# maryambabaei/hybrid-FEM-LSSVR

Measured on AMD Instinct MI355X. Metric: LSSVR-enhanced elements/sec, 1D Poisson deg-8/16-pt, higher is better.
Workload: dtype f64

## Files before the change

### __graft_entry__.py

```python
from __future__ import annotations

import os
import subprocess
import sys

ROOT = os.path.dirname(os.path.abspath(__file__))
if ROOT not in sys.path:
    sys.path.insert(0, ROOT)

CSRC = os.path.join(ROOT, "hybrid_fem_lssvr_amd", "csrc")


def build() -> None:
    if os.environ.get("LSSVR_HIP_LIB"):
        raise RuntimeError("LSSVR_HIP_LIB is set: build(), the tests and the benchmark use the one "
                           "in-tree library only (the override is for scripts/ A/B experiments)")
    env = dict(os.environ)
    env.setdefault("HIPCC", "/opt/rocm/bin/hipcc")
    subprocess.run(["make", "-C", CSRC, "-j", str(min(8, os.cpu_count() or 1))], check=True, env=env)
    subprocess.run(["make", "-C", CSRC, "demo"], check=True, env=env)
    subprocess.run(["make", "-C", CSRC, "check-dpp"], check=True, env=env)
    import hybrid_fem_lssvr_amd as pkg
    lib = pkg._capi.load()
    assert pkg._capi.LIB_PATH == pkg._capi.IN_TREE_LIB
    assert lib.lssvr_version() == pkg._capi.ABI_VERSION
    import oracle.lssvr_oracle


def smoke() -> None:
    import numpy as np
    import torch
    import hybrid_fem_lssvr_amd as pkg
    from oracle import lssvr_oracle as orc

    if not torch.cuda.is_available():
        raise RuntimeError("smoke() needs cuda:0 (MI355X); there is no CPU fallback")
    solver = pkg.FEMLSSVRPrimalSolver(25, lssvr_M=9, lssvr_gamma=1e4, global_domain=(-1, 1),
                                      n_colloc=16)
    solver.solve()
    nodes = np.linspace(-1, 1, 25)
    u_ref = orc.fem_p1_solve(nodes)
    assert np.max(np.abs(solver.fem_values - u_ref)) < 1e-13, "P1 solve mismatch"
    W = np.array([f.coef for f in solver.lssvr_functions])
    W_ref = orc.enhance_all_vec(nodes, solver.fem_values, 9, 1e4, 16)
    err = orc.rel_l2_coef(W, W_ref).max()
    assert err < 1e-12, f"enhance mismatch {err}"
    xq = np.linspace(-1, 1, 201)
    uq = solver.evaluate_solution(xq)
    uo, eo = orc.evaluate_solution(nodes, W, xq)
    assert np.max(np.abs(uq - uo)) < 1e-14, "evaluate mismatch"
    assert np.array_equal(solver.element_indices(xq), eo), "element index mismatch"
    l2 = np.linalg.norm(uq - orc.true_solution(xq)) / np.linalg.norm(orc.true_solution(xq))
    big = pkg.enhance_elements(nodes, solver.fem_values, 33, 1e4, n_colloc=64)
    Wb = big.W.cpu().numpy()
    Wb_ref = orc.enhance_all_vec(nodes, solver.fem_values, 33, 1e4, 64)
    errb = orc.rel_l2_coef(Wb, Wb_ref).max()
    assert errb < 1e-11, f"degree-32 mismatch {errb}"
    print(f"smoke ok: deg8 rel-L2 vs oracle {err:.2e}, deg32 {errb:.2e}, "
          f"hybrid rel-L2 error vs sin(pi x) {l2:.3e}")


if __name__ == "__main__":
    build()
    if len(sys.argv) > 1 and sys.argv[1] == "smoke":
        smoke()
```

### hybrid_fem_lssvr_amd/csrc/capi.hip

```cpp
#include <cstdarg>
#include <vector>
#include <cstdio>
#include <cstring>

#include <new>
#include "lssvr_kernels.hpp"

namespace {

thread_local char g_err[256] = {0};

int fail(int code, const char* fmt, ...) {
  va_list ap;
  va_start(ap, fmt);
  vsnprintf(g_err, sizeof(g_err), fmt, ap);
  va_end(ap);
  return code;
}

int check_launch(hipError_t e, const char* what) {
  if (e == hipSuccess) return LSSVR_OK;
  return fail(LSSVR_ERR_LAUNCH, "%s: %s", what, hipGetErrorString(e));
}

int check_ne(int64_t ne, int ne_min = 1, const char* why = "") {
  if (ne < ne_min) return fail(LSSVR_ERR_SIZE, "ne = %lld < %d%s", (long long)ne, ne_min, why);
  if (ne > (int64_t)1 << 40) return fail(LSSVR_ERR_SIZE, "ne = %lld too large", (long long)ne);
  return LSSVR_OK;
}

bool is_finite(double v) { return v > -INFINITY && v < INFINITY; }

int check_layout(int table_layout) {
  if (table_layout != LSSVR_TABLE_ELEMENT_MAJOR && table_layout != LSSVR_TABLE_POINT_MAJOR)
    return fail(LSSVR_ERR_SIZE, "unknown table_layout %d", table_layout);
  return LSSVR_OK;
}

int check_kinds(int kind_left, int kind_right) {
  if ((kind_left != LSSVR_END_DIRICHLET && kind_left != LSSVR_END_ROBIN) ||
      (kind_right != LSSVR_END_DIRICHLET && kind_right != LSSVR_END_ROBIN))
    return fail(LSSVR_ERR_SIZE, "end kinds (%d, %d) must be LSSVR_END_DIRICHLET or LSSVR_END_ROBIN", kind_left,
                kind_right);
  return LSSVR_OK;
}

int check_nl_kind(int kind, int nterm) {
  if (kind != LSSVR_NL_POLY && kind != LSSVR_NL_EXP)
    return fail(LSSVR_ERR_RHS, "unknown kind %d (LSSVR_NL_POLY or LSSVR_NL_EXP)", kind);
  if (kind == LSSVR_NL_POLY && (nterm < 1 || nterm > 6))
    return fail(LSSVR_ERR_SIZE, "nterm = %d outside [1, 6]", nterm);
  if (kind == LSSVR_NL_EXP && nterm != 2) return fail(LSSVR_ERR_SIZE, "nterm = %d: LSSVR_NL_EXP has q_0 and q_1", nterm);
  return LSSVR_OK;
}

int bind_enhance(lssvr::EnhanceArgs& a, const double* x, const double* u, int64_t ne, int64_t elem_offset,
                 int64_t ne_global, double gxmin, double gxmax, double bc_left, double bc_right, int M,
                 int n_colloc, double gamma, double* W, int32_t* status, int32_t* fail_count) {
  if (ne < 0) return fail(LSSVR_ERR_SIZE, "ne = %lld < 0", (long long)ne);
  if (ne > 0 && (!x || !u || !W)) return fail(LSSVR_ERR_NULL, "x, u and W must be non-NULL");
  if (elem_offset < 0 || ne_global < elem_offset + ne)
    return fail(LSSVR_ERR_SIZE, "shard [%lld, %lld) does not fit ne_global = %lld",
                (long long)elem_offset, (long long)(elem_offset + ne), (long long)ne_global);
  if (M < 2 || M > lssvr::kLargeMaxM)
    return fail(LSSVR_ERR_DEGREE, "M = %d outside [2, %d]", M, lssvr::kLargeMaxM);
  if (n_colloc < 2 || n_colloc > 4096)
    return fail(LSSVR_ERR_SIZE, "n_colloc = %d outside [2, 4096]", n_colloc);
  if (!(gamma > 0.0)) return fail(LSSVR_ERR_SIZE, "gamma must be > 0");
  if (ne * (int64_t)M / M != ne) return fail(LSSVR_ERR_SIZE, "ne*M overflows");
  a = lssvr::EnhanceArgs{};
  a.x = x;
  a.u = u;
  a.ne = ne;
  a.ne_mesh = ne;
  a.elem_offset = elem_offset;
  a.ne_global = ne_global;
  a.gxmin = gxmin;
  a.gxmax = gxmax;
  a.bc_left = bc_left;
  a.bc_right = bc_right;
  a.gamma = gamma;
  a.inv_gamma = 1.0 / gamma;
// ... 260 lines not shown

int colloc_points_entry(const double* x, int64_t ne, int n_colloc, double* xc, void* stream, bool point_major) {
  if (ne < 0) return fail(LSSVR_ERR_SIZE, "ne < 0");
  if (n_colloc < 2) return fail(LSSVR_ERR_SIZE, "n_colloc < 2");
  if (ne > 0 && (!x || !xc)) return fail(LSSVR_ERR_NULL, "x and xc must be non-NULL");
  return check_launch(lssvr::colloc_points(x, ne, n_colloc, xc, reinterpret_cast<hipStream_t>(stream), point_major),
                      point_major ? "colloc_points(point-major)" : "colloc_points");
}

}

extern "C" {

int lssvr_version(void) { return LSSVR_ABI_VERSION; }

const char* lssvr_last_error(void) { return g_err; }

int lssvr_enhance(const double* x, const double* u, int64_t ne, int64_t elem_offset,
                  int64_t ne_global, double gxmin, double gxmax, double bc_left, double bc_right,
                  int M, int n_colloc, double gamma, int rhs_id, const double* rhs_params_host,
                  const double* rhs_values, int solver_id, double* W, int32_t* status,
                  int32_t* fail_count, void* stream) {
  return lssvr_enhance_ws(x, u, ne, elem_offset, ne_global, gxmin, gxmax, bc_left, bc_right, M, n_colloc, gamma,
                          rhs_id, rhs_params_host, rhs_values, solver_id, W, status, fail_count, nullptr, 0, stream,
                          nullptr);
}

int64_t lssvr_enhance_work_bytes(int64_t ne, int M, int n_colloc, int solver_id) {
  if (ne <= 0) return 0;
  if (solver_id == LSSVR_SOLVER_PRIMAL_MOMENT) return lssvr::enhance_moment_ws_bytes(ne, M, n_colloc);
  if (solver_id != LSSVR_SOLVER_PRIMAL || M <= lssvr::kSmallMaxM) return 0;
  return lssvr::enhance_moment_ws_bytes(ne, M, n_colloc);
}

int lssvr_enhance_ws(const double* x, const double* u, int64_t ne, int64_t elem_offset,
                     int64_t ne_global, double gxmin, double gxmax, double bc_left, double bc_right,
                     int M, int n_colloc, double gamma, int rhs_id, const double* rhs_params_host,
                     const double* rhs_values, int solver_id, double* W, int32_t* status,
                     int32_t* fail_count, void* work, int64_t work_bytes, void* stream,
                     float* kernel_ms_host) {
  lssvr::EnhanceArgs a;
  const int rc = bind_enhance_ws(a, x, u, ne, elem_offset, ne_global, gxmin, gxmax, bc_left, bc_right, M, n_colloc,
                                 gamma, rhs_id, rhs_params_host, rhs_values, solver_id, W, status, fail_count, work,
                                 work_bytes);
  if (rc != LSSVR_OK || ne == 0) return rc;
  hipStream_t s = reinterpret_cast<hipStream_t>(stream);
  return timed_launch([&](const lssvr::LaunchOpts* o) { return enhance_dispatch(a, solver_id, s, o, work, work_bytes); },
                      kernel_ms_host);
}

int lssvr_enhance_ws_sequence(const double* x, const double* u, int64_t ne, int64_t elem_offset,
                              int64_t ne_global, double gxmin, double gxmax, double bc_left, double bc_right,
                              int M, int n_colloc, double gamma, int rhs_id, const double* rhs_params_host,
                              const double* rhs_values, int solver_id, double* W, int32_t* status,
                              int32_t* fail_count, void* work, int64_t work_bytes, void* stream,
                              int repeats, float* kernel_ms_host) {
  lssvr::EnhanceArgs a;
  int rc = check_sequence(ne, repeats, kernel_ms_host);
  if (rc == LSSVR_OK)
    rc = bind_enhance_ws(a, x, u, ne, elem_offset, ne_global, gxmin, gxmax, bc_left, bc_right, M, n_colloc, gamma,
                         rhs_id, rhs_params_host, rhs_values, solver_id, W, status, fail_count, work, work_bytes);
  if (rc != LSSVR_OK) return rc;
  hipStream_t s = reinterpret_cast<hipStream_t>(stream);
  return timed_sequence([&](const lssvr::LaunchOpts* o) { return enhance_dispatch(a, solver_id, s, o, work, work_bytes); },
                        s, repeats, kernel_ms_host);
}

int lssvr_enhance_profiled(const double* x, const double* u, int64_t ne, int64_t elem_offset,
                           int64_t ne_global, double gxmin, double gxmax, double bc_left,
                           double bc_right, int M, int n_colloc, double gamma, int rhs_id,
                           const double* rhs_params_host, const double* rhs_values, int solver_id,
                           double* W, int32_t* status, void* stream, float* kernel_ms_host) {
  if (!kernel_ms_host) return fail(LSSVR_ERR_NULL, "kernel_ms_host must be non-NULL");
  if (ne < 1) return fail(LSSVR_ERR_SIZE, "nothing to profile: ne = %lld", (long long)ne);
  return lssvr_enhance_ws(x, u, ne, elem_offset, ne_global, gxmin, gxmax, bc_left, bc_right, M, n_colloc, gamma,
                          rhs_id, rhs_params_host, rhs_values, solver_id, W, status, nullptr, nullptr, 0, stream,
                          kernel_ms_host);
}

struct lssvr_step_plan {
  lssvr::EnhanceArgs a;
  lssvr::P1Args p;
  const double* memo = nullptr;
};

static int64_t step_memo_bytes(const lssvr_step_plan& b) {
  const lssvr::EnhanceArgs& a = b.a;
  if (a.M > lssvr::kSmallMaxM || a.refine > 0 || a.gamma_values || a.rhs_id != LSSVR_RHS_SIN || a.ne < 1) return 0;
  return 8 * lssvr::step_memo_doubles(a.M, a.ne);
}

static int bind_step(lssvr_step_plan& b, const double* x, const double* u, int64_t ne, int64_t elem_offset,
                     int64_t ne_global, double gxmin, double gxmax, double bc_left, double bc_right,
                     int M, int n_colloc, double gamma, const double* rhs_params_host, int nquad,
                     double* diag, double* off, double* load, double* W, int32_t* status,
                     int32_t* fail_count) {
  lssvr::EnhanceArgs& a = b.a;
  int rc = bind_enhance(a, x, u, ne, elem_offset, ne_global, gxmin, gxmax, bc_left, bc_right, M, n_colloc, gamma,
                        W, status, fail_count);
  if (rc != LSSVR_OK) return rc;
  if (ne < 1) return fail(LSSVR_ERR_SIZE, "ne = %lld < 1", (long long)ne);
  rc = bind_p1(b.p, x, ne, nquad, diag, off, load);
  if (rc == LSSVR_OK) rc = bind_rhs(a, LSSVR_RHS_SIN, rhs_params_host, nullptr, false, "ne");
  if (rc != LSSVR_OK) return rc;
  if (n_colloc < M - 2)
    return fail(LSSVR_ERR_SOLVER, "lssvr_step: n_colloc = %d < M-2 = %d: the primal normal equations are "
                                  "rank deficient; use lssvr_p1_assemble + lssvr_enhance (dual solver)",
                n_colloc, M - 2);
  return bind_p1_rhs(b.p, LSSVR_RHS_SIN, rhs_params_host, nullptr);
}

static int run_step(const lssvr_step_plan& b, hipStream_t s) {
  const lssvr::EnhanceArgs& a = b.a;
  const lssvr::P1Args& p = b.p;
  if (a.M <= lssvr::kSmallMaxM && a.refine == 0)
    return check_launch(lssvr::step_small(a, p, s, nullptr, b.memo), "step_small");
  int rc = check_launch(lssvr::p1_assemble(p, s), "p1_assemble");
  if (rc != LSSVR_OK) return rc;
  if (a.M <= lssvr::kSmallMaxM) return check_launch(lssvr::enhance_small(a, s), "enhance_small(refine)");
  return check_launch(lssvr::enhance_large(a, s), "enhance_large");
}

int lssvr_step(const double* x, const double* u, int64_t ne, int64_t elem_offset,
               int64_t ne_global, double gxmin, double gxmax, double bc_left, double bc_right,
               int M, int n_colloc, double gamma, const double* rhs_params_host, int nquad,
               double* diag, double* off, double* load, double* W, int32_t* status,
               int32_t* fail_count, void* stream) {
  lssvr_step_plan b;
  const int rc = bind_step(b, x, u, ne, elem_offset, ne_global, gxmin, gxmax, bc_left, bc_right, M, n_colloc,
                           gamma, rhs_params_host, nquad, diag, off, load, W, status, fail_count);
  if (rc != LSSVR_OK) return rc;
  return run_step(b, reinterpret_cast<hipStream_t>(stream));
}

int lssvr_step_plan_create(lssvr_step_plan** plan, const double* x, const double* u, int64_t ne,
                           int64_t elem_offset, int64_t ne_global, double gxmin, double gxmax,
                           double bc_left, double bc_right, int M, int n_colloc, double gamma,
                           const double* rhs_params_host, int nquad, double* diag, double* off,
                           double* load, double* W, int32_t* status, int32_t* fail_count) {
  if (!plan) return fail(LSSVR_ERR_NULL, "plan must be non-NULL");
  *plan = nullptr;
  lssvr_step_plan* b = new (std::nothrow) lssvr_step_plan;
  if (!b) return fail(LSSVR_ERR_LAUNCH, "out of host memory");
  const int rc = bind_step(*b, x, u, ne, elem_offset, ne_global, gxmin, gxmax, bc_left, bc_right, M, n_colloc,
                           gamma, rhs_params_host, nquad, diag, off, load, W, status, fail_count);
  if (rc != LSSVR_OK) {
    delete b;
    return rc;
  }
  *plan = b;
  return LSSVR_OK;
}

int lssvr_step_plan_launch(const lssvr_step_plan* plan, void* stream) {
  if (!plan) return fail(LSSVR_ERR_NULL, "plan must be non-NULL");
  return run_step(*plan, reinterpret_cast<hipStream_t>(stream));
}

int64_t lssvr_step_plan_memo_bytes(const lssvr_step_plan* plan) { return plan ? step_memo_bytes(*plan) : 0; }

int lssvr_step_plan_memo_bind(lssvr_step_plan* plan, void* memo, int64_t memo_bytes, void* stream) {
  if (!plan) return fail(LSSVR_ERR_NULL, "plan must be non-NULL");
  if (!memo) {
    plan->memo = nullptr;
    return LSSVR_OK;
  }
  const int64_t need = step_memo_bytes(*plan);
  if (need == 0)
    return fail(LSSVR_ERR_SOLVER, "this plan cannot use a memo (lssvr_step_plan_memo_bytes is 0: M = %d, n_colloc = %d)",
                plan->a.M, plan->a.n);
  if (memo_bytes < need)
    return fail(LSSVR_ERR_SIZE, "memo_bytes = %lld < lssvr_step_plan_memo_bytes = %lld", (long long)memo_bytes,
                (long long)need);
  if (reinterpret_cast<uintptr_t>(memo) % 8 != 0) return fail(LSSVR_ERR_SIZE, "memo must be 8-byte aligned");
  plan->memo = nullptr;
  const int rc = check_launch(lssvr::step_small_memo_fill(plan->a, static_cast<double*>(memo),
                                                          reinterpret_cast<hipStream_t>(stream)),
                              "step_memo_fill");
  if (rc == LSSVR_OK) plan->memo = static_cast<const double*>(memo);
  return rc;
}

int lssvr_step_plan_destroy(lssvr_step_plan* plan) {
  delete plan;
  return LSSVR_OK;
}

int lssvr_enhance_varcoef(const double* x, const double* u, int64_t ne, int64_t elem_offset,
                          int64_t ne_global, double gxmin, double gxmax, double bc_left,
                          double bc_right, int M, int n_colloc, double gamma,
                          const double* a_values, const double* da_values,
                          const double* rhs_values, double* W, int32_t* status,
                          int32_t* fail_count, void* stream) {
  return lssvr_enhance_varcoef_ws(x, u, ne, elem_offset, ne_global, gxmin, gxmax, bc_left, bc_right, M,
                                  n_colloc, gamma, a_values, da_values, rhs_values, LSSVR_TABLE_ELEMENT_MAJOR,
                                  W, status, fail_count, nullptr, 0, stream, nullptr);
}

int lssvr_step_varcoef(const double* x, const double* u, int64_t ne, int64_t elem_offset,
                       int64_t ne_global, double gxmin, double gxmax, double bc_left, double bc_right,
                       int M, int n_colloc, double gamma, const double* a_values,
                       const double* da_values, const double* rhs_values, int table_layout, int nquad,
                       const double* rhs_quad, const double* a_quad, double* diag, double* off,
                       double* load, double* W, int32_t* status, int32_t* fail_count, void* stream) {
  lssvr::EnhanceArgs a;
  int rc = bind_enhance(a, x, u, ne, elem_offset, ne_global, gxmin, gxmax, bc_left, bc_right, M, n_colloc, gamma,
                        W, status, fail_count);
  if (rc != LSSVR_OK) return rc;
  if (ne < 1) return fail(LSSVR_ERR_SIZE, "ne = %lld < 1", (long long)ne);
  rc = bind_varcoef(a, a_values, da_values, rhs_values, table_layout, true);
  if (rc != LSSVR_OK) return rc;
  if (!rhs_quad || !a_quad) return fail(LSSVR_ERR_NULL, "rhs_quad and a_quad must be non-NULL");
  lssvr::P1Args p;
  rc = bind_p1(p, x, ne, nquad, diag, off, load);
  if (rc != LSSVR_OK) return rc;
  if (n_colloc < M - 2)
    return fail(LSSVR_ERR_SOLVER, "lssvr_step_varcoef: n_colloc = %d < M-2 = %d: use lssvr_p1_assemble + "
                                  "lssvr_enhance_varcoef (dual solver)", n_colloc, M - 2);
  p.rhs_id = LSSVR_RHS_ARRAY;
  p.rhs_quad = rhs_quad;
  p.a_quad = a_quad;
  hipStream_t s = reinterpret_cast<hipStream_t>(stream);
  if (M <= lssvr::kStepVarcoefFusedMaxM) return check_launch(lssvr::step_small_vc(a, p, s), "step_small_vc");
  rc = check_launch(lssvr::p1_assemble(p, s), "p1_assemble");
  if (rc != LSSVR_OK) return rc;
  return enhance_dispatch(a, LSSVR_SOLVER_PRIMAL, s, nullptr);
}

int lssvr_enhance_react(const double* x, const double* u, int64_t ne, int64_t elem_offset,
                        int64_t ne_global, double gxmin, double gxmax, double bc_left,
                        double bc_right, int M, int n_colloc, double gamma,
                        const double* a_values, const double* da_values, const double* c_values,
                        const double* rhs_values, double* W, int32_t* status,
                        int32_t* fail_count, void* stream) {
  return lssvr_enhance_react_ws(x, u, ne, elem_offset, ne_global, gxmin, gxmax, bc_left, bc_right, M,
                                n_colloc, gamma, a_values, da_values, c_values, rhs_values,
                                LSSVR_TABLE_ELEMENT_MAJOR, W, status, fail_count, nullptr, 0, stream, nullptr);
}

int lssvr_enhance_react_ws(const double* x, const double* u, int64_t ne, int64_t elem_offset,
                           int64_t ne_global, double gxmin, double gxmax, double bc_left,
                           double bc_right, int M, int n_colloc, double gamma,
                           const double* a_values, const double* da_values, const double* c_values,
                           const double* rhs_values, int table_layout, double* W, int32_t* status,
                           int32_t* fail_count, void* work, int64_t work_bytes, void* stream,
                           float* kernel_ms_host) {
  lssvr::EnhanceReactArgs a;
  const int rc = bind_react_ws(a, x, u, ne, elem_offset, ne_global, gxmin, gxmax, bc_left, bc_right, M, n_colloc,
                               gamma, a_values, da_values, c_values, rhs_values, table_layout, W, status,
                               fail_count, work, work_bytes);
  if (rc != LSSVR_OK || ne == 0) return rc;
  hipStream_t s = reinterpret_cast<hipStream_t>(stream);
  return timed_launch([&](const lssvr::LaunchOpts* o) { return react_dispatch(a, s, o); }, kernel_ms_host);
}

int lssvr_enhance_multi(const double* x, const double* u, int64_t ne, int64_t elem_offset,
                        int64_t ne_global, double gxmin, double gxmax, const double* bc_values, int ncases,
                        int M, int n_colloc, double gamma, const double* a_values, const double* da_values,
                        const double* c_values, const double* rhs_values, int table_layout, double* W,
                        int32_t* status, int32_t* fail_count, void* stream, float* kernel_ms_host) {
  lssvr::EnhanceMultiArgs a{};
  int rc = bind_varcoef_ws(a, x, u, ne, elem_offset, ne_global, gxmin, gxmax, 0.0, 0.0, M, n_colloc, gamma,
// ... 1332 lines not shown
```

### hybrid_fem_lssvr_amd/csrc/enhance_small.hip

```cpp
#include "lssvr_kernels.hpp"
#include "lssvr_p1.hpp"

namespace lssvr {

#define LSSVR_DECLARE_SMALL_RANGE(NAME)                                                          \
  hipError_t enhance_small_##NAME(const EnhanceArgs& a, hipStream_t s, const LaunchOpts* o);     \
  hipError_t step_small_##NAME(const EnhanceArgs& e, const P1Args& a, const QuadRule& q,         \
                               hipStream_t s, const LaunchOpts* o, const double* memo);          \
  hipError_t step_memo_fill_##NAME(const EnhanceArgs& e, double* memo, hipStream_t s);           \
  hipError_t step_small_vc_##NAME(const EnhanceArgs& e, const P1Args& a, const QuadRule& q,      \
                                  hipStream_t s, const LaunchOpts* o);
LSSVR_DECLARE_SMALL_RANGE(a)
LSSVR_DECLARE_SMALL_RANGE(b)
LSSVR_DECLARE_SMALL_RANGE(c)
LSSVR_DECLARE_SMALL_RANGE(d)

hipError_t enhance_small(const EnhanceArgs& a, hipStream_t s, const LaunchOpts* o) {
  if (a.M <= 10) return enhance_small_a(a, s, o);
  if (a.M <= 15) return enhance_small_b(a, s, o);
  if (a.M <= 19) return enhance_small_c(a, s, o);
  return enhance_small_d(a, s, o);
}

hipError_t step_small(const EnhanceArgs& e, const P1Args& a, hipStream_t s, const LaunchOpts* o,
                      const double* memo) {
  QuadRule q;
  if (!quad_rule(a.nquad, q)) return hipErrorInvalidValue;
  if (e.M <= 10) return step_small_a(e, a, q, s, o, memo);
  if (e.M <= 15) return step_small_b(e, a, q, s, o, memo);
  if (e.M <= 19) return step_small_c(e, a, q, s, o, memo);
  return step_small_d(e, a, q, s, o, memo);
}

hipError_t step_small_memo_fill(const EnhanceArgs& e, double* memo, hipStream_t s) {
  if (e.M <= 10) return step_memo_fill_a(e, memo, s);
  if (e.M <= 15) return step_memo_fill_b(e, memo, s);
  if (e.M <= 19) return step_memo_fill_c(e, memo, s);
  return step_memo_fill_d(e, memo, s);
}

hipError_t step_small_vc(const EnhanceArgs& e, const P1Args& a, hipStream_t s, const LaunchOpts* o) {
  QuadRule q;
  if (!quad_rule(a.nquad, q)) return hipErrorInvalidValue;
  if (e.M <= 10) return step_small_vc_a(e, a, q, s, o);
  if (e.M <= 15) return step_small_vc_b(e, a, q, s, o);
  return hipErrorInvalidValue;
}

}
```

### hybrid_fem_lssvr_amd/csrc/enhance_small_impl.hpp

```cpp
#pragma once
#include "enhance_small_cheb.hpp"
#include "lssvr_device.hpp"
#include "lssvr_kernels.hpp"
#include "lssvr_p1.hpp"

namespace lssvr {

constexpr int kStageK = 8;
constexpr int kStageArr = 64 * (kStageK + 1);
template <int M, int RHS, bool VC, bool RX = false>
constexpr int kSmallTilePerWave =
    (RHS == LSSVR_RHS_ARRAY && (VC ? (RX ? 4 : 3) : 1) * kStageArr > 64 * M) ? (VC ? (RX ? 4 : 3) : 1) * kStageArr
                                                                             : 64 * M;
constexpr int kPrefetch = 4;
constexpr int kPrefetchReact = 2;

template <int M, int RHS, bool VC, bool RX = false, typename Args = EnhanceArgs>
__device__ __forceinline__ void enhance_small_body(const Args& p, const unsigned block,
                                                   double* __restrict__ tile) {
  static_assert(!RX || VC, "reaction rows extend the variable-coefficient rows");
  constexpr int MR = M - 2;
  constexpr int NT = MR * (MR + 1) / 2;

  const int tid = threadIdx.x;
// ... 331 lines not shown
    if (i <= a.ne) p1_node<true>(a, q, i);
  }
}

template <int M>
__global__ __launch_bounds__(kBlock) void step_memo_fill_kernel(EnhanceArgs p, double* memo) {
  if constexpr (M == 2) {
    const int64_t e = (int64_t)blockIdx.x * kBlock + threadIdx.x;
    if (e < p.ne) {
      memo[e] = p.x[e];
      if (e == p.ne - 1) memo[e + 1] = p.x[e + 1];
    }
  } else {
    enhance_small_body_cheb<M, LSSVR_RHS_SIN, false, NoProbe, MemoFill>(p, blockIdx.x, nullptr, NoProbe{}, MemoFill{memo});
  }
}

constexpr int kStepVcMaxM = 12;
template <int M, int RHS>
__global__ __launch_bounds__(kBlock) void step_small_vc_kernel(EnhanceArgs p, P1Args a, QuadRule q,
                                                                unsigned eblocks) {
  __shared__ double tile[(kBlock / 64) * kSmallTilePerWave<M, RHS, true>];
  if (blockIdx.x < eblocks) {
    enhance_small_body<M, RHS, true>(p, blockIdx.x, tile);
  } else {
    const int64_t i = (int64_t)(blockIdx.x - eblocks) * kBlock + threadIdx.x;
    if (i <= a.ne) p1_node<false>(a, q, i);
  }
}

template <int M, int RHS, bool VC>
static hipError_t launch_small(const EnhanceArgs& a, hipStream_t s, const LaunchOpts* o) {
  const unsigned blocks = (unsigned)((a.ne + kBlock - 1) / kBlock);
  if constexpr (!VC && M >= kRefineMinM) {
    if (a.refine > 0) return launch(enhance_small_refine_kernel<M, RHS>, dim3(blocks), dim3(kBlock), s, o, a);
  }
  return launch(enhance_small_kernel<M, RHS, VC, 1>, dim3(blocks), dim3(kBlock), s, o, a);
}

template <int M>
static hipError_t launch_step(const EnhanceArgs& e, const P1Args& a, const QuadRule& q,
                              hipStream_t s, const LaunchOpts* o, const double* memo) {
  const unsigned eb = (unsigned)((e.ne + kBlock - 1) / kBlock);
  const unsigned ab = (unsigned)((a.ne + 1 + kBlock - 1) / kBlock);
  return launch(step_small_kernel<M>, dim3(eb + ab), dim3(kBlock), s, o, e, a, q, eb, memo);
}

template <int M>
static hipError_t launch_memo_fill(const EnhanceArgs& e, double* memo, hipStream_t s) {
  const unsigned eb = (unsigned)((e.ne + kBlock - 1) / kBlock);
  return launch(step_memo_fill_kernel<M>, dim3(eb), dim3(kBlock), s, nullptr, e, memo);
}

template <int M>
static hipError_t launch_step_vc(const EnhanceArgs& e, const P1Args& a, const QuadRule& q,
                                 hipStream_t s, const LaunchOpts* o) {
  if constexpr (M <= kStepVcMaxM) {
    const unsigned eb = (unsigned)((e.ne + kBlock - 1) / kBlock);
    const unsigned ab = (unsigned)((a.ne + 1 + kBlock - 1) / kBlock);
    if (e.tab_ps != 1)
      return launch(step_small_vc_kernel<M, LSSVR_RHS_ARRAY_PM>, dim3(eb + ab), dim3(kBlock), s, o, e, a, q, eb);
    return launch(step_small_vc_kernel<M, LSSVR_RHS_ARRAY>, dim3(eb + ab), dim3(kBlock), s, o, e, a, q, eb);
  } else {
    return hipErrorInvalidValue;
  }
}

#define LSSVR_DEFINE_SMALL_RANGE(NAME, FOR_EACH_M)                                              \
  hipError_t enhance_small_##NAME(const EnhanceArgs& a, hipStream_t s, const LaunchOpts* o) {    \
    switch (a.M) {                                                                               \
      FOR_EACH_M(LSSVR_SMALL_CASE_ENH)                                                           \
      default:                                                                                   \
        return hipErrorInvalidValue;                                                             \
    }                                                                                            \
  }                                                                                              \
  hipError_t step_small_##NAME(const EnhanceArgs& e, const P1Args& a, const QuadRule& q,         \
                               hipStream_t s, const LaunchOpts* o, const double* memo) {         \
    switch (e.M) {                                                                               \
      FOR_EACH_M(LSSVR_SMALL_CASE_STEP)                                                          \
      default:                                                                                   \
        return hipErrorInvalidValue;                                                             \
    }                                                                                            \
  }                                                                                              \
  hipError_t step_memo_fill_##NAME(const EnhanceArgs& e, double* memo, hipStream_t s) {          \
    switch (e.M) {                                                                               \
      FOR_EACH_M(LSSVR_SMALL_CASE_MEMO_FILL)                                                     \
      default:                                                                                   \
        return hipErrorInvalidValue;                                                             \
    }                                                                                            \
  }                                                                                              \
  hipError_t step_small_vc_##NAME(const EnhanceArgs& e, const P1Args& a, const QuadRule& q,      \
                                  hipStream_t s, const LaunchOpts* o) {                          \
    switch (e.M) {                                                                               \
      FOR_EACH_M(LSSVR_SMALL_CASE_STEP_VC)                                                       \
      default:                                                                                   \
        return hipErrorInvalidValue;                                                             \
    }                                                                                            \
  }

#define LSSVR_SMALL_CASE_ENH(MM)                                                     \
  case MM:                                                                           \
    if (a.a_values && a.tab_ps != 1) return launch_small<MM, LSSVR_RHS_ARRAY_PM, true>(a, s, o); \
    if (a.a_values) return launch_small<MM, LSSVR_RHS_ARRAY, true>(a, s, o);         \
    if (a.rhs_id == LSSVR_RHS_SIN) return launch_small<MM, LSSVR_RHS_SIN, false>(a, s, o); \
    if (a.tab_ps != 1) return launch_small<MM, LSSVR_RHS_ARRAY_PM, false>(a, s, o);  \
    return launch_small<MM, LSSVR_RHS_ARRAY, false>(a, s, o);
#define LSSVR_SMALL_CASE_REACT(MM)                                                                          \
  case MM: {                                                                                                \
    const unsigned blocks = (unsigned)((a.ne + kBlock - 1) / kBlock);                                       \
    if (a.tab_ps != 1)                                                                                      \
      return launch(enhance_small_react_kernel<MM, LSSVR_RHS_ARRAY_PM>, dim3(blocks), dim3(kBlock), s, o, a); \
    return launch(enhance_small_react_kernel<MM, LSSVR_RHS_ARRAY>, dim3(blocks), dim3(kBlock), s, o, a);    \
  }
#define LSSVR_SMALL_CASE_STEP(MM) \
  case MM:                        \
    return launch_step<MM>(e, a, q, s, o, memo);
#define LSSVR_SMALL_CASE_MEMO_FILL(MM) \
  case MM:                             \
    return launch_memo_fill<MM>(e, memo, s);
#define LSSVR_SMALL_CASE_STEP_VC(MM) \
  case MM:                           \
    return launch_step_vc<MM>(e, a, q, s, o);

}
```

### hybrid_fem_lssvr_amd/csrc/lssvr_kernels.hpp

```cpp
#pragma once
#include <hip/hip_runtime.h>
#include <hip/hip_ext.h>
#include <stdint.h>
#include "../../include/lssvr_hip.h"
#include "../../include/lssvr_hip_bench.h"
#include "lssvr_device.hpp"

namespace lssvr {

constexpr int kSmallMaxM = 22;
constexpr int64_t kWriteThroughMaxDoubles = int64_t(1) << 21;
constexpr int kLargeMaxM = 33;

struct EnhanceArgs {
  const double* x;
  const double* u;
  int64_t ne, elem_offset, ne_global;
  double gxmin, gxmax, bc_left, bc_right, gamma;
  double inv_gamma;
  int M, n;
  int refine;
  int rhs_id;
  double rhs_amp, rhs_omega;
  const double* rhs_values;
  const double* a_values;
  const double* da_values;
  int64_t tab_es, tab_ps;
  const int64_t* elem_ids;
  int64_t ne_mesh;
  const double* gamma_values;
  int64_t ldw;
  double* W;
  int32_t* status;
  int32_t* fail_count;
  TrigTables trig;
};

struct EnhanceReactArgs : EnhanceArgs {
  const double* c_values;
};

struct EnhanceMultiArgs : EnhanceReactArgs {
  const double* bc_values;
  int nc;
};

struct LaunchOpts {
  hipEvent_t start = nullptr;
  hipEvent_t stop = nullptr;
};

template <typename K, typename... Args>
inline hipError_t launch(K kernel, dim3 grid, dim3 block, hipStream_t s, const LaunchOpts* o,
                         Args... args) {
  if (o && (o->start || o->stop))
    hipExtLaunchKernelGGL(kernel, grid, block, 0, s, o->start, o->stop, 0, args...);
  else
    hipLaunchKernelGGL(kernel, grid, block, 0, s, args...);
  return hipGetLastError();
}

inline unsigned xcd_count() {
  static thread_local int cached_dev = -1;
  static thread_local unsigned cached = 1;
  int dev = 0;
  if (hipGetDevice(&dev) != hipSuccess) return 1;
  if (dev != cached_dev) {
    int v = 0;
    if (hipDeviceGetAttribute(&v, hipDeviceAttributeNumberOfXccs, dev) != hipSuccess || v < 1) v = 1;
    cached = (unsigned)v;
    cached_dev = dev;
  }
  return cached;
}

inline unsigned cu_count() {
  static thread_local int cached_dev = -1;
  static thread_local unsigned cached = 1;
  int dev = 0;
  if (hipGetDevice(&dev) != hipSuccess) return 1;
  if (dev != cached_dev) {
    int v = 0;
    if (hipDeviceGetAttribute(&v, hipDeviceAttributeMultiprocessorCount, dev) != hipSuccess || v < 1) v = 1;
    cached = (unsigned)v;
    cached_dev = dev;
  }
  return cached;
}

hipError_t enhance_small(const EnhanceArgs& a, hipStream_t s, const LaunchOpts* o = nullptr);
hipError_t enhance_large(const EnhanceArgs& a, hipStream_t s, const LaunchOpts* o = nullptr);
constexpr int kReactSmallMaxM = 16;
hipError_t enhance_small_react(const EnhanceReactArgs& a, hipStream_t s, const LaunchOpts* o = nullptr);
hipError_t enhance_large_react(const EnhanceReactArgs& a, hipStream_t s, const LaunchOpts* o = nullptr);
int enhance_multi_rc(int M);
hipError_t enhance_multi(const EnhanceMultiArgs& a, int ncases, hipStream_t s, const LaunchOpts* o = nullptr);
int enhance_refine_steps(int M, int n);
int enhance_small_refine_steps(int M, int n);
int64_t enhance_moment_ws_bytes(int64_t ne, int M, int n);
hipError_t enhance_large_split(const EnhanceArgs& a, void* work, hipStream_t s, const LaunchOpts* o = nullptr);
constexpr int kMomentWsStride = 96;
bool enhance_parity_applies(int M, int n);
hipError_t launch_solve4_parity(const EnhanceArgs& a, const double* ws, hipStream_t s, const LaunchOpts* o);
hipError_t enhance_dual(const EnhanceArgs& a, hipStream_t s, const LaunchOpts* o = nullptr);
constexpr int kSharedMaxM = 33;
hipError_t enhance_shared(const EnhanceArgs& a, const double* op, hipStream_t s,
                          const LaunchOpts* o = nullptr);

hipError_t colloc_points(const double* x, int64_t ne, int n, double* xc, hipStream_t s, bool point_major = false);
hipError_t colloc_points_subset(const double* x, int64_t ne_mesh, const int64_t* ids, int64_t nsub, int n, double* xc,
                                hipStream_t s, bool point_major);

struct QuadRule {
  double xi[5];
  double wt[5];
};

struct P1Args {
  const double* x;
  int64_t ne;
  int nquad;
  int rhs_id;
  double rhs_amp, rhs_omega;
  const double* rhs_quad;
  const double* a_quad;
  double* diag;
  double* off;
  double* load;
  double* kloc;
  double* floc;
};
hipError_t p1_assemble(const P1Args& a, hipStream_t s);
struct P1ReactArgs : P1Args {
  const double* c_quad;
};
hipError_t p1_assemble_react(const P1ReactArgs& a, hipStream_t s);
struct P1ConvArgs : P1ReactArgs {
  const double* b_quad;
  double* sub;
  double* sup;
};
hipError_t p1_assemble_conv(const P1ConvArgs& a, hipStream_t s);
hipError_t step_small(const EnhanceArgs& e, const P1Args& a, hipStream_t s,
                      const LaunchOpts* o = nullptr, const double* memo = nullptr);
__host__ __device__ constexpr int step_memo_planes(int M) { return M > 2 ? 3 * (M - 2) - 2 : 0; }
__host__ __device__ constexpr int64_t step_memo_ne_pad(int64_t ne) { return (ne + 63) & ~(int64_t)63; }
constexpr int64_t step_memo_doubles(int M, int64_t ne) { return step_memo_planes(M) * step_memo_ne_pad(ne) + ne + 1; }
hipError_t step_small_memo_fill(const EnhanceArgs& e, double* memo, hipStream_t s);
constexpr int kStepVarcoefFusedMaxM = 12;
hipError_t step_small_vc(const EnhanceArgs& e, const P1Args& a, hipStream_t s, const LaunchOpts* o = nullptr);
hipError_t quad_points(const double* x, int64_t ne, int nquad, double* xq, hipStream_t s);

constexpr int kTriMultiCases = 8;
int64_t tridiag_multi_work_bytes(int64_t ne, int nc);
int64_t tridiag_work_bytes(int64_t ne);
hipError_t tridiag_dirichlet_solve(const double* diag, const double* off, const double* load, int64_t ne, int nc,
                                   const double* bc, double u0, double u1, double* u, void* work, hipStream_t s);
hipError_t tridiag_ns_dirichlet_solve(const double* diag, const double* sub, const double* sup, const double* load,
                                      int64_t ne, int nc, const double* bc, double u0, double u1, double* u,
                                      void* work, hipStream_t s);
int64_t tridiag_bc_work_bytes(int64_t ne, int nc);
hipError_t tridiag_bc_solve(const double* diag, const double* off, const double* load, int64_t ne, int nc, bool f0,
                            bool f1, double k0, double k1, const double* bc, double* u, void* work, hipStream_t s);
hipError_t tridiag_ns_bc_solve(const double* diag, const double* sub, const double* sup, const double* load,
                               int64_t ne, int nc, bool f0, bool f1, double k0, double k1, const double* bc,
                               double* u, void* work, hipStream_t s);
int64_t tridiag_periodic_work_bytes(int64_t ne, int nc);
hipError_t tridiag_periodic_solve(const double* diag, const double* off, const double* load, int64_t ne, int nc,
                                  double* u, void* work, hipStream_t s);
hipError_t tridiag_ns_periodic_solve(const double* diag, const double* sub, const double* sup, const double* load,
                                     int64_t ne, int nc, double* u, void* work, hipStream_t s);
int64_t tridiag_pivot_work_bytes(int64_t ne, int nc);
hipError_t tridiag_pivot_solve(const double* diag, const double* sub, const double* sup, const double* load,
                               int64_t ne, int nc, bool f0, bool f1, double k0, double k1, const double* bc,
                               double* u, int32_t* info, void* work, hipStream_t s);
void tridiag_pivot_host(const double* diag, const double* sub, const double* sup, const double* load, int64_t ne,
                        int nc, bool f0, bool f1, double k0, double k1, const double* bc, double* u, int32_t* info);
hipError_t p1_load_multi(const double* x, int64_t ne, int nquad, const double* rhs_quad, int nc, double* load,
                         hipStream_t s);

int64_t flux_work_bytes(int64_t ne);
hipError_t flux_dirichlet_solve(const double* kloc, const double* load, int64_t ne, double u0,
                                double u1, double* u, void* work, hipStream_t s);

hipError_t eval_points(const double* x, const double* W, int64_t ne, int M, const double* xq,
                       int64_t P, double* uq, int64_t* elem, hipStream_t s);

hipError_t flux_aggregate(const double* kloc, const double* load, int64_t ne, bool first_global,
                          void* work, double* agg3, hipStream_t s);
hipError_t flux_finish(const double* kloc, const double* load, int64_t ne, bool first_global,
                       bool last_global, const void* work, const double* prefix3,
                       const double* grand3, double u0, double u1, double* u, hipStream_t s);

hipError_t eval_error(const double* x, const double* W, int64_t ne, int M, const double* xq,
                      int64_t P, double amp, double omega, double* out, hipStream_t s);

constexpr int kAdaptMaxNq = 32;
constexpr int kAdaptMaxM = 33;
struct GaussRuleN {
  double xi[kAdaptMaxNq];
  double wt[kAdaptMaxNq];
};
struct EstimateArgs {
  const double* x;
  const double* W;
  int64_t ne;
  int M, nq, ms;
  double rhs_amp, rhs_omega;
  const double* rhs_values;
  double* eta2;
  double* jump;
  double* work;
};
struct EstimateVcArgs : EstimateArgs {
  const double* a_values;
  const double* da_values;
  const double* a_ends;
};
struct EstimateReactArgs : EstimateVcArgs {
  const double* c_values;
};
bool gauss_rule(int nq, double* xi, double* wt);
int64_t adapt_work_bytes(int64_t ne);
hipError_t eval_deriv(const double* x, const double* W, int64_t ne, int M, int order, const double* xq,
                      int64_t P, double* out, int64_t* elem, hipStream_t s);
hipError_t estimate_points(const double* x, int64_t ne, int nq, double* xq, hipStream_t s);
hipError_t estimate(EstimateArgs a, int rhs_mode, double* out3, hipStream_t s);
// ... 237 lines not shown
```

### hybrid_fem_lssvr_amd/ops.py

```python
from __future__ import annotations

import collections
import contextlib
import ctypes
import math
import os
import threading

import numpy as np
import torch

from . import _capi
from ._capi import (RHS_ARRAY, RHS_ARRAY_PM, RHS_SIN, SOLVER_DUAL, SOLVER_PRIMAL,
                    SOLVER_PRIMAL_MOMENT, SOLVER_PRIMAL_WAVE, TABLE_ELEMENT_MAJOR, TABLE_POINT_MAJOR)

SOLVER_SHARED = 100

POISSON_AMP = float(math.pi ** 2)
POISSON_OMEGA = float(math.pi)


def _dev(t, name, dtype=torch.float64):
    if not isinstance(t, torch.Tensor):
        raise TypeError(f"{name}: expected a torch.Tensor device buffer, got {type(t).__name__}")
# ... 231 lines not shown
    else:
        nsub = ne
    if gamma_values is not None:
        _dev(gamma_values, "gamma_values")
        if gamma_values.numel() != ne:
            raise ValueError("gamma_values must hold one value per mesh element")
    if status is not None:
        _dev(status, "status", torch.int32)
        if status.numel() != ne:
            raise ValueError("status is indexed by mesh element: int32[ne]")
    _check_fail_count(fail_count)
    rhs_id, params = _rhs(rhs, rhs_values, nsub * n_colloc, "nsub*n_colloc", point_major)
    pre = _prefix(x, u, elem_offset, ne_global, global_domain, bc, M, n_colloc, gamma)
    with _work_arg(work, lib, x, nsub, M, n_colloc, SOLVER_PRIMAL, stream) as wk:
        rc = lib.lssvr_enhance_subset_ws(*pre[:3], _ptr(elem_ids), int(nsub), *pre[3:],
                                         _ptr(gamma_values), rhs_id, params, _ptr(rhs_values),
                                         _ptr(W), int(W.shape[1]), _ptr(status), _ptr(fail_count),
                                         _ptr(wk), 0 if wk is None else wk.numel() * 8, _stream(stream))
    _capi.check(rc, "lssvr_enhance_subset_ws")
    return W


def build_shared_operator(h, M, gamma, n_colloc, *, device="cuda:0", stream=None):
    n = int(n_colloc)
    h = float(h)
    nel = n + 2
    nodes = (torch.arange(nel + 1, dtype=torch.float64) - 0.5 * nel) * h
    scl = 2.0 / float(nodes[1] - nodes[0])
    f = torch.zeros((nel, n), dtype=torch.float64)
    f[torch.arange(n), torch.arange(n)] = scl * scl
    uu = torch.zeros(nel + 1, dtype=torch.float64)
    uu[n + 1] = 1.0
    x = nodes.to(device)
    W, st = enhance(x, uu.to(device), int(M), float(gamma), n, rhs_values=f.to(device),
                    elem_offset=1, ne_global=nel + 2, global_domain=(float(nodes[0]) - h, float(nodes[-1]) + h),
                    stream=stream)
    op = torch.empty((nel, M), dtype=torch.float64, device=device)
    op[:n] = W[:n]
    op[n] = W[n + 1]
    op[n + 1] = W[n]
    if int(st.sum().item()) != 0:
        raise _capi.LssvrHipError("build_shared_operator: the canonical element's factorisation broke down")
    return op


def enhance_shared(x, u, op, M, n_colloc, *, rhs=(POISSON_AMP, POISSON_OMEGA), rhs_values=None,
                   elem_offset=0, ne_global=None, global_domain, bc=(0.0, 0.0), out=None, status=None,
                   fail_count=None, stream=None, profiled=False, point_major=False):
    lib = _capi.load()
    ne, ne_global = _shard(x, u, elem_offset, ne_global)
    _dev(op, "op")
    if op.dim() != 2 or op.shape[0] != n_colloc + 2 or op.shape[1] != M or not op.is_contiguous():
        raise ValueError("op must be a contiguous float64[(n_colloc+2), M] tensor")
    out, status = _check_buffers(ne, M, n_colloc, x, out=out, status=status, fail_count=fail_count)
    rhs_id, params = _rhs(rhs, rhs_values, ne * n_colloc, "ne*n_colloc", point_major)
    args = _prefix(x, u, elem_offset, ne_global, global_domain, bc, M, n_colloc, 1.0)[:-1] + (
        rhs_id, params, _ptr(rhs_values), _ptr(op), _ptr(out), _ptr(status), _ptr(fail_count), _stream(stream))
    if profiled:
        return _timed(lib, "lssvr_enhance_shared", args)
    _capi.check(lib.lssvr_enhance_shared(*args, None), "lssvr_enhance_shared")
    return out, status


def enhance_profiled(x, u, M, gamma, n_colloc=12, *, rhs=(POISSON_AMP, POISSON_OMEGA),
                     elem_offset=0, ne_global=None, global_domain, bc=(0.0, 0.0),
                     solver=SOLVER_PRIMAL, out=None, status=None, stream=None, work=None, repeats=None):
    lib = _capi.load()
    ne, ne_global = _shard(x, u, elem_offset, ne_global)
    out, status = _check_buffers(ne, M, n_colloc, x, out=out, status=status)
    with _work_arg(work, lib, x, ne, M, n_colloc, solver, stream) as wk:
        args = _prefix(x, u, elem_offset, ne_global, global_domain, bc, M, n_colloc, gamma) + (
            RHS_SIN, _capi.rhs_params(*rhs), None, int(solver), _ptr(out), _ptr(status), None,
            _ptr(wk), 0 if wk is None else wk.numel() * 8, _stream(stream))
        return _timed(lib, "lssvr_enhance_ws", args, repeats)


def _bind(lib, name, args):
    argtypes = _capi.SIGNATURES[name][1]
    ready = (ctypes.Array, ctypes._SimpleCData, ctypes._Pointer, type(ctypes.byref(ctypes.c_int())))
    conv = tuple(a if (a is None or isinstance(a, ready)) else tp(a) for tp, a in zip(argtypes, args))
    return getattr(lib, name), conv


STEP_MEMO_DEFAULT = os.environ.get("LSSVR_STEP_MEMO", "1") != "0"
STEP_MEMO_MAX_BYTES = int(os.environ.get("LSSVR_STEP_MEMO_MAX_BYTES", 208 << 20))


class StepPlan:

    def __init__(self, x, u, M, gamma, n_colloc=12, *, rhs=(POISSON_AMP, POISSON_OMEGA), nquad=2,
                 elem_offset=0, ne_global=None, global_domain, bc=(0.0, 0.0), bands=None,
                 out=None, status=None, fail_count=None, memo=None):
        self.lib = _capi.load()
        ne, ne_global = _shard(x, u, elem_offset, ne_global)
        self.bands = _bands(x, ne, bands)
        self.W, self.status = _check_buffers(ne, M, n_colloc, x, out=out, status=status,
                                             fail_count=fail_count)
        self.fail_count = fail_count
        nb = int(self.lib.lssvr_enhance_work_bytes(ne, int(M), int(n_colloc), SOLVER_PRIMAL))
        self._work = torch.empty((nb + 7) // 8, dtype=torch.float64, device=x.device) if nb > 0 else None
        self._keep = (x, u, _capi.rhs_params(*rhs))
        pre = _prefix(x, u, elem_offset, ne_global, global_domain, bc, M, n_colloc, gamma)
        bands = (_ptr(self.bands["diag"]), _ptr(self.bands["off"]), _ptr(self.bands["load"]))
        outs = (_ptr(self.W), _ptr(self.status), _ptr(fail_count))
        self._args = pre + (self._keep[2], int(nquad)) + bands + outs
        self._step, self._cargs = _bind(self.lib, "lssvr_step", self._args)
        self._handle = ctypes.c_void_p()
        create, cargs = _bind(self.lib, "lssvr_step_plan_create", (ctypes.byref(self._handle),) + self._args)
        rc = create(*cargs)
        if rc < 0:
            self._handle = None
            _capi.check(rc, "lssvr_step_plan_create")
        self._launch = self.lib.lssvr_step_plan_launch
        self._memo = None
        self.memo_bytes = 0
        if (STEP_MEMO_DEFAULT if memo is None else memo) and self._work is None:
            nb = int(self.lib.lssvr_step_plan_memo_bytes(self._handle))
            if 0 < nb <= STEP_MEMO_MAX_BYTES:
                self._memo = torch.empty(nb // 8, dtype=torch.float64, device=x.device)
                self.memo_bytes = nb
                self.refresh_memo()
                torch.cuda.current_stream(x.device).synchronize()

        if self._work is not None:
            self._asm_args = (_ptr(x), ne, int(nquad), RHS_SIN, self._keep[2], None, None) + bands + (None, None)
            self._enh_args = pre + (RHS_SIN, self._keep[2], None, SOLVER_PRIMAL) + outs + (
                _ptr(self._work), self._work.numel() * 8)

    def launch(self, stream=None):
        st = _stream(stream)
        if self._work is not None:
            rc = self.lib.lssvr_p1_assemble(*self._asm_args, st)
            if rc >= 0:
                rc = self.lib.lssvr_enhance_ws(*self._enh_args, st, None)
        else:
            rc = self._launch(self._handle, st)
        if rc < 0:
            _capi.check(rc, "lssvr_step")
        return self.W, self.status

    def refresh_memo(self, stream=None):
        if self._memo is None:
            return
        st = _stream(torch.cuda.current_stream(self._memo.device) if stream is None else stream)
        _capi.check(self.lib.lssvr_step_plan_memo_bind(self._handle, _ptr(self._memo), self.memo_bytes, st),
                    "lssvr_step_plan_memo_bind")

    def __del__(self):
        h = getattr(self, "_handle", None)
        if h:
            try:
                self.lib.lssvr_step_plan_destroy(h)
            except Exception:
                pass
            self._handle = None


def enhance_varcoef(x, u, M, gamma, n_colloc, a_values, da_values, rhs_values, *, elem_offset=0,
                    ne_global=None, global_domain=None, bc=(0.0, 0.0), out=None, status=None,
                    fail_count=None, stream=None, profiled=False, point_major=False, repeats=None,
                    c_values=None, b_values=None):
    lib = _capi.load()
    ne, ne_global = _shard(x, u, elem_offset, ne_global)
    da_values = _fold(da_values, b_values)
    _tables(ne, n_colloc, a_values=a_values, da_values=da_values, rhs_values=rhs_values,
            **({} if c_values is None else {"c_values": c_values}))
    if c_values is not None and repeats is not None:
        raise ValueError("repeats is not available with c_values (lssvr_enhance_react_ws has no sequence form)")
    pre = _prefix(x, u, elem_offset, ne_global, global_domain, bc, M, n_colloc, gamma)
    out, status = _check_buffers(ne, M, n_colloc, x, out=out, status=status, fail_count=fail_count)
    kind, tabs = _variant(a_values, da_values, rhs_values, c_values)
    name = f"lssvr_enhance_{kind}_ws"
    args = pre + tabs + (_layout(point_major), _ptr(out), _ptr(status), _ptr(fail_count), None, 0, _stream(stream))
    if profiled:
        return _timed(lib, name, args, repeats)
    _capi.check(getattr(lib, name)(*args, None), name)
    return out, status


def _elem_list(elem_ids, ne, x):
    if elem_ids is None:
        return ne
    _dev(elem_ids, "elem_ids", torch.int64)
    if elem_ids.dim() != 1 or elem_ids.numel() > ne:
        raise ValueError(f"elem_ids must be int64[nsub <= ne = {ne}], got {list(elem_ids.shape)}")
    if elem_ids.device != x.device:
        raise RuntimeError(f"elem_ids lives on {elem_ids.device}, x on {x.device}")
    return elem_ids.numel()


def enhance_varcoef_subset(x, u, M, gamma, n_colloc, W, a_values, da_values, rhs_values, *, elem_ids=None,
                           gamma_values=None, c_values=None, b_values=None, point_major=False, elem_offset=0,
                           ne_global=None, global_domain, bc=(0.0, 0.0), status=None, fail_count=None, stream=None):
    lib = _capi.load()
    M, n_colloc = int(M), int(n_colloc)
    ne, ne_global = _shard(x, u, elem_offset, ne_global)
    _dev(W, "W")
    if W.dim() != 2 or W.shape[0] != ne or W.shape[1] < M:
        raise ValueError("W must be a contiguous float64[ne, ldw >= M] tensor")
    nsub = _elem_list(elem_ids, ne, x)
    da_values = _fold(da_values, b_values)
    named = dict(a_values=a_values, da_values=da_values, rhs_values=rhs_values)
    if c_values is not None:
        named["c_values"] = c_values
    _tables(nsub, n_colloc, **named)
    if gamma_values is not None:
        _dev(gamma_values, "gamma_values")
        if gamma_values.numel() != ne:
            raise ValueError("gamma_values must hold one value per mesh element")
    if status is not None:
        _dev(status, "status", torch.int32)
        if status.numel() != ne:
            raise ValueError("status is indexed by mesh element: int32[ne]")
    _check_fail_count(fail_count)
    _same_device(x, u=u, W=W, gamma_values=gamma_values, status=status, fail_count=fail_count, **named)
    pre = _prefix(x, u, elem_offset, ne_global, global_domain, bc, M, n_colloc, gamma)
    rc = lib.lssvr_enhance_react_subset(*pre[:3], _ptr(elem_ids), int(nsub), *pre[3:], _ptr(gamma_values),
                                        _ptr(a_values), _ptr(da_values), _ptr(c_values), _ptr(rhs_values),
                                        _layout(point_major), _ptr(W), int(W.shape[1]), _ptr(status),
# ... 1361 lines not shown
```

Baseline: 18.05 billion.

## Prerecord step kernel launch and add a CPython fast-call launch entry

At plan creation the step path now records the kernel symbol, grid and a packed argument block. Each launch then goes through hipModuleLaunchKernel with a cached per-device function handle instead of re-dispatching through the templated launch path. A small C extension calls lssvr_step_plan_launch directly from Python with METH_FASTCALL, bypassing ctypes argument conversion. This targets per-launch host overhead for small workloads, and adds a dependence on the kernarg layout matching the struct, guarded by static_asserts.

```diff
diff --git a/__graft_entry__.py b/__graft_entry__.py
--- a/__graft_entry__.py
+++ b/__graft_entry__.py
@@ -17,6 +17,7 @@
                            "in-tree library only (the override is for scripts/ A/B experiments)")
     env = dict(os.environ)
     env.setdefault("HIPCC", "/opt/rocm/bin/hipcc")
+    env.setdefault("PYTHON", sys.executable)
     subprocess.run(["make", "-C", CSRC, "-j", str(min(8, os.cpu_count() or 1))], check=True, env=env)
     subprocess.run(["make", "-C", CSRC, "demo"], check=True, env=env)
     subprocess.run(["make", "-C", CSRC, "check-dpp"], check=True, env=env)
diff --git a/hybrid_fem_lssvr_amd/csrc/capi.hip b/hybrid_fem_lssvr_amd/csrc/capi.hip
--- a/hybrid_fem_lssvr_amd/csrc/capi.hip
+++ b/hybrid_fem_lssvr_amd/csrc/capi.hip
@@ -1,3 +1,4 @@
+#include <atomic>
 #include <cstdarg>
 #include <vector>
 #include <cstdio>
@@ -424,6 +425,9 @@
   lssvr::EnhanceArgs a;
   lssvr::P1Args p;
   const double* memo = nullptr;
+  static constexpr int kMaxDevices = 64;
+  lssvr::StepRecord rec;
+  mutable std::atomic<hipFunction_t> fn[kMaxDevices] = {};
 };
 
 static int64_t step_memo_bytes(const lssvr_step_plan& b) {
@@ -452,9 +456,29 @@
   return bind_p1_rhs(b.p, LSSVR_RHS_SIN, rhs_params_host, nullptr);
 }
 
+static int run_step_record(const lssvr_step_plan& b, hipStream_t s) {
+  int dev = 0;
+  hipError_t e = hipGetDevice(&dev);
+  if (e != hipSuccess) return check_launch(e, "step_small");
+  if (dev < 0 || dev >= lssvr_step_plan::kMaxDevices)
+    return check_launch(lssvr::step_small(b.a, b.p, s, nullptr, b.memo), "step_small");
+  hipFunction_t f = b.fn[dev].load(std::memory_order_acquire);
+  if (!f) {
+    e = hipGetFuncBySymbol(&f, b.rec.symbol);
+    if (e != hipSuccess) return check_launch(e, "step_small (hipGetFuncBySymbol)");
+    b.fn[dev].store(f, std::memory_order_release);
+  }
+  size_t bytes = sizeof(lssvr::StepKernelArgs);
+  void* extra[] = {HIP_LAUNCH_PARAM_BUFFER_POINTER, const_cast<lssvr::StepKernelArgs*>(&b.rec.args),
+                   HIP_LAUNCH_PARAM_BUFFER_SIZE, &bytes, HIP_LAUNCH_PARAM_END};
+  return check_launch(hipModuleLaunchKernel(f, b.rec.grid, 1, 1, lssvr::kBlock, 1, 1, 0, s, nullptr, extra),
+                      "step_small");
+}
+
 static int run_step(const lssvr_step_plan& b, hipStream_t s) {
   const lssvr::EnhanceArgs& a = b.a;
   const lssvr::P1Args& p = b.p;
+  if (b.rec.symbol) return run_step_record(b, s);
   if (a.M <= lssvr::kSmallMaxM && a.refine == 0)
     return check_launch(lssvr::step_small(a, p, s, nullptr, b.memo), "step_small");
   int rc = check_launch(lssvr::p1_assemble(p, s), "p1_assemble");
@@ -490,6 +514,7 @@
     delete b;
     return rc;
   }
+  if (b->a.M <= lssvr::kSmallMaxM && b->a.refine == 0) lssvr::step_small_record(b->a, b->p, nullptr, b->rec);
   *plan = b;
   return LSSVR_OK;
 }
@@ -505,6 +530,7 @@
   if (!plan) return fail(LSSVR_ERR_NULL, "plan must be non-NULL");
   if (!memo) {
     plan->memo = nullptr;
+    plan->rec.args.memo = nullptr;
     return LSSVR_OK;
   }
   const int64_t need = step_memo_bytes(*plan);
@@ -516,10 +542,11 @@
                 (long long)need);
   if (reinterpret_cast<uintptr_t>(memo) % 8 != 0) return fail(LSSVR_ERR_SIZE, "memo must be 8-byte aligned");
   plan->memo = nullptr;
+  plan->rec.args.memo = nullptr;
   const int rc = check_launch(lssvr::step_small_memo_fill(plan->a, static_cast<double*>(memo),
                                                           reinterpret_cast<hipStream_t>(stream)),
                               "step_memo_fill");
-  if (rc == LSSVR_OK) plan->memo = static_cast<const double*>(memo);
+  if (rc == LSSVR_OK) plan->memo = plan->rec.args.memo = static_cast<const double*>(memo);
   return rc;
 }
 
diff --git a/hybrid_fem_lssvr_amd/csrc/enhance_small.hip b/hybrid_fem_lssvr_amd/csrc/enhance_small.hip
--- a/hybrid_fem_lssvr_amd/csrc/enhance_small.hip
+++ b/hybrid_fem_lssvr_amd/csrc/enhance_small.hip
@@ -7,6 +7,7 @@
   hipError_t enhance_small_##NAME(const EnhanceArgs& a, hipStream_t s, const LaunchOpts* o);     \
   hipError_t step_small_##NAME(const EnhanceArgs& e, const P1Args& a, const QuadRule& q,         \
                                hipStream_t s, const LaunchOpts* o, const double* memo);          \
+  const void* step_small_symbol_##NAME(int M);                                                   \
   hipError_t step_memo_fill_##NAME(const EnhanceArgs& e, double* memo, hipStream_t s);           \
   hipError_t step_small_vc_##NAME(const EnhanceArgs& e, const P1Args& a, const QuadRule& q,      \
                                   hipStream_t s, const LaunchOpts* o);
@@ -32,6 +33,27 @@
   return step_small_d(e, a, q, s, o, memo);
 }
 
+bool step_small_record(const EnhanceArgs& e, const P1Args& a, const double* memo, StepRecord& r) {
+  r = StepRecord{};
+  QuadRule q;
+  if (e.M < 2 || e.M > kSmallMaxM || e.ne < 1 || !quad_rule(a.nquad, q)) return false;
+  const void* symbol = e.M <= 10 ? step_small_symbol_a(e.M)
+                     : e.M <= 15 ? step_small_symbol_b(e.M)
+                     : e.M <= 19 ? step_small_symbol_c(e.M)
+                                 : step_small_symbol_d(e.M);
+  if (!symbol) return false;
+  const unsigned eb = (unsigned)((e.ne + kBlock - 1) / kBlock);
+  const unsigned ab = (unsigned)((a.ne + 1 + kBlock - 1) / kBlock);
+  r.grid = eb + ab;
+  r.args.p = e;
+  r.args.a = a;
+  r.args.q = q;
+  r.args.eblocks = eb;
+  r.args.memo = memo;
+  r.symbol = symbol;
+  return true;
+}
+
 hipError_t step_small_memo_fill(const EnhanceArgs& e, double* memo, hipStream_t s) {
   if (e.M <= 10) return step_memo_fill_a(e, memo, s);
   if (e.M <= 15) return step_memo_fill_b(e, memo, s);
diff --git a/hybrid_fem_lssvr_amd/csrc/enhance_small_impl.hpp b/hybrid_fem_lssvr_amd/csrc/enhance_small_impl.hpp
--- a/hybrid_fem_lssvr_amd/csrc/enhance_small_impl.hpp
+++ b/hybrid_fem_lssvr_amd/csrc/enhance_small_impl.hpp
@@ -437,6 +437,13 @@
         return hipErrorInvalidValue;                                                             \
     }                                                                                            \
   }                                                                                              \
+  const void* step_small_symbol_##NAME(int M) {                                                  \
+    switch (M) {                                                                                 \
+      FOR_EACH_M(LSSVR_SMALL_CASE_STEP_SYMBOL)                                                   \
+      default:                                                                                   \
+        return nullptr;                                                                          \
+    }                                                                                            \
+  }                                                                                              \
   hipError_t step_memo_fill_##NAME(const EnhanceArgs& e, double* memo, hipStream_t s) {          \
     switch (e.M) {                                                                               \
       FOR_EACH_M(LSSVR_SMALL_CASE_MEMO_FILL)                                                     \
@@ -470,6 +477,9 @@
 #define LSSVR_SMALL_CASE_STEP(MM) \
   case MM:                        \
     return launch_step<MM>(e, a, q, s, o, memo);
+#define LSSVR_SMALL_CASE_STEP_SYMBOL(MM) \
+  case MM:                               \
+    return reinterpret_cast<const void*>(&step_small_kernel<MM>);
 #define LSSVR_SMALL_CASE_MEMO_FILL(MM) \
   case MM:                             \
     return launch_memo_fill<MM>(e, memo, s);
diff --git a/hybrid_fem_lssvr_amd/csrc/lssvr_kernels.hpp b/hybrid_fem_lssvr_amd/csrc/lssvr_kernels.hpp
--- a/hybrid_fem_lssvr_amd/csrc/lssvr_kernels.hpp
+++ b/hybrid_fem_lssvr_amd/csrc/lssvr_kernels.hpp
@@ -2,6 +2,8 @@
 #include <hip/hip_runtime.h>
 #include <hip/hip_ext.h>
 #include <stdint.h>
+#include <cstddef>
+#include <type_traits>
 #include "../../include/lssvr_hip.h"
 #include "../../include/lssvr_hip_bench.h"
 #include "lssvr_device.hpp"
@@ -143,6 +145,34 @@
 hipError_t p1_assemble_conv(const P1ConvArgs& a, hipStream_t s);
 hipError_t step_small(const EnhanceArgs& e, const P1Args& a, hipStream_t s,
                       const LaunchOpts* o = nullptr, const double* memo = nullptr);
+struct StepKernelArgs {
+  EnhanceArgs p;
+  P1Args a;
+  QuadRule q;
+  unsigned eblocks;
+  const double* memo;
+};
+constexpr size_t kernarg_offset(size_t prev_end, size_t align) { return (prev_end + align - 1) / align * align; }
+static_assert(std::is_trivially_copyable<StepKernelArgs>::value && std::is_standard_layout<StepKernelArgs>::value,
+              "the block is copied byte for byte into the kernel-argument segment");
+static_assert(offsetof(StepKernelArgs, p) == 0, "step_small_kernel: p");
+static_assert(offsetof(StepKernelArgs, a) == kernarg_offset(sizeof(EnhanceArgs), alignof(P1Args)),
+              "step_small_kernel: a");
+static_assert(offsetof(StepKernelArgs, q) ==
+                  kernarg_offset(offsetof(StepKernelArgs, a) + sizeof(P1Args), alignof(QuadRule)),
+              "step_small_kernel: q");
+static_assert(offsetof(StepKernelArgs, eblocks) ==
+                  kernarg_offset(offsetof(StepKernelArgs, q) + sizeof(QuadRule), alignof(unsigned)),
+              "step_small_kernel: eblocks");
+static_assert(offsetof(StepKernelArgs, memo) ==
+                  kernarg_offset(offsetof(StepKernelArgs, eblocks) + sizeof(unsigned), alignof(const double*)),
+              "step_small_kernel: memo");
+struct StepRecord {
+  const void* symbol = nullptr;
+  unsigned grid = 0;
+  StepKernelArgs args;
+};
+bool step_small_record(const EnhanceArgs& e, const P1Args& a, const double* memo, StepRecord& r);
 __host__ __device__ constexpr int step_memo_planes(int M) { return M > 2 ? 3 * (M - 2) - 2 : 0; }
 __host__ __device__ constexpr int64_t step_memo_ne_pad(int64_t ne) { return (ne + 63) & ~(int64_t)63; }
 constexpr int64_t step_memo_doubles(int M, int64_t ne) { return step_memo_planes(M) * step_memo_ne_pad(ne) + ne + 1; }
diff --git a/hybrid_fem_lssvr_amd/csrc/steplaunch.c b/hybrid_fem_lssvr_amd/csrc/steplaunch.c
--- /dev/null
+++ b/hybrid_fem_lssvr_amd/csrc/steplaunch.c
@@ -0,0 +1,34 @@
+#define PY_SSIZE_T_CLEAN
+#include <Python.h>
+
+#include "../../include/lssvr_hip.h"
+
+static PyObject* steplaunch_launch(PyObject* self, PyObject* const* args, Py_ssize_t nargs) {
+  (void)self;
+  if (nargs != 2) {
+    PyErr_SetString(PyExc_TypeError, "launch(handle, stream) takes exactly two integers");
+    return NULL;
+  }
+  void* plan = PyLong_AsVoidPtr(args[0]);
+  if (!plan && PyErr_Occurred()) return NULL;
+  void* stream = PyLong_AsVoidPtr(args[1]);
+  if (!stream && PyErr_Occurred()) return NULL;
+  return PyLong_FromLong(lssvr_step_plan_launch((const lssvr_step_plan*)plan, stream));
+}
+
+static PyMethodDef steplaunch_methods[] = {
+    {"launch", (PyCFunction)(void (*)(void))steplaunch_launch, METH_FASTCALL,
+     "launch(handle, stream) -> int: lssvr_step_plan_launch on the plan handle and the raw stream handle"},
+    {NULL, NULL, 0, NULL}};
+
+static struct PyModuleDef steplaunch_module = {PyModuleDef_HEAD_INIT, "_steplaunch",
+                                               "direct entry for lssvr_step_plan_launch", -1, steplaunch_methods,
+                                               NULL, NULL, NULL, NULL};
+
+PyMODINIT_FUNC PyInit__steplaunch(void) {
+  if (lssvr_version() != LSSVR_ABI_VERSION) {
+    PyErr_SetString(PyExc_ImportError, "_steplaunch: liblssvr_hip.so has another ABI version");
+    return NULL;
+  }
+  return PyModule_Create(&steplaunch_module);
+}
diff --git a/hybrid_fem_lssvr_amd/ops.py b/hybrid_fem_lssvr_amd/ops.py
--- a/hybrid_fem_lssvr_amd/ops.py
+++ b/hybrid_fem_lssvr_amd/ops.py
@@ -337,6 +337,22 @@
     return getattr(lib, name), conv
 
 
+_FAST_LAUNCH = []
+
+
+def _fast_launch():
+    if not _FAST_LAUNCH:
+        fn = None
+        if os.environ.get("LSSVR_STEP_FASTCALL", "1") != "0" and _capi.LIB_PATH == _capi.IN_TREE_LIB:
+            try:
+                from . import _steplaunch
+                fn = _steplaunch.launch
+            except ImportError:
+                fn = None
+        _FAST_LAUNCH.append(fn)
+    return _FAST_LAUNCH[0]
+
+
 STEP_MEMO_DEFAULT = os.environ.get("LSSVR_STEP_MEMO", "1") != "0"
 STEP_MEMO_MAX_BYTES = int(os.environ.get("LSSVR_STEP_MEMO_MAX_BYTES", 208 << 20))
 
@@ -366,7 +382,10 @@
         if rc < 0:
             self._handle = None
             _capi.check(rc, "lssvr_step_plan_create")
-        self._launch = self.lib.lssvr_step_plan_launch
+        self._launch, self._h = self.lib.lssvr_step_plan_launch, self._handle
+        fast = _fast_launch()
+        if fast is not None:
+            self._launch, self._h = fast, int(self._handle.value)
         self._memo = None
         self.memo_bytes = 0
         if (STEP_MEMO_DEFAULT if memo is None else memo) and self._work is None:
@@ -389,7 +408,7 @@
             if rc >= 0:
                 rc = self.lib.lssvr_enhance_ws(*self._enh_args, st, None)
         else:
-            rc = self._launch(self._handle, st)
+            rc = self._launch(self._h, st)
         if rc < 0:
             _capi.check(rc, "lssvr_step")
         return self.W, self.status
```

Measured after the change: 17.43 billion. 3.4% lower.
